# jankammeth/BA-path-planning

Hardware: AMD Instinct MI355X
Metric: SCP iterations/sec (N agents x K waypoints) (higher is better)
Workload: dtype f64

## Files before the change

ba-path-planning_amd/csrc/scp_common.h:

```cpp
#pragma once
#include <hip/hip_runtime.h>

#include <cstdarg>
#include <cstdint>
#include <cstdio>
#include <cstring>

#include "scp_hip.h"

struct scp_stats_mirror {
  scp_pair_stats stats;
  unsigned long long n_spec;
  double pts[6];
  double rel[64];
  volatile unsigned long long seq;
};

constexpr int SCP_SMALL_MAX_WG = 2048;

struct scp_ctx {
  int device;
  int n_cu;
  hipStream_t stream;
  char err[512];
// ... 35 lines not shown
    va_end(ap);
  }
  return code;
}

#define SCP_HIP_CHECK(ctx, call)                                                                     \
  do {                                                                                               \
    hipError_t e_ = (call);                                                                          \
    if (e_ != hipSuccess)                                                                            \
      return scp_fail((ctx), SCP_ERR_HIP, "%s failed: %s (%s:%d)", #call, hipGetErrorString(e_),    \
                      __FILE__, __LINE__);                                                           \
  } while (0)

#define SCP_REQUIRE(ctx, cond, ...)                                   \
  do {                                                                \
    if (!(cond)) return scp_fail((ctx), SCP_ERR_INVALID, __VA_ARGS__); \
  } while (0)

static inline int64_t scp_pairs(int N) { return (int64_t)N * (N - 1) / 2; }
static inline int scp_cdiv(int64_t a, int64_t b) { return (int)((a + b - 1) / b); }

hipError_t scp_raise_lds_limit(int device, const void* kernel, size_t bytes);

bool scp_wait_host_word(volatile unsigned long long* word, unsigned long long seq, int timeout_s);

int scp_ctx_wait_stats(scp_ctx* ctx, scp_pair_stats* out);

int scp_violations_from_solution(scp_ctx* ctx, int N, int K, int D, double R, double h, int64_t q_begin, int64_t q_end,
                                 const double* pos_prev, const double* x_tm, const double* p0, const double* v0, double* x_out,
                                 double* pos_out, double feas_tol, int64_t* new_rows, int64_t new_cap, uint32_t* sel_bitmap,
                                 scp_pair_stats* stats, const double* rel_prev ,
                                 int64_t* spec_rows , int64_t spec_cap,
                                 uint32_t* spec_bitmap, double spec_margin, bool* fused);
void scp_ctx_mirror_rel(scp_ctx* ctx, int64_t n, double* out);
int scp_select_from_solution(scp_ctx* ctx, int N, int K, int D, double R, double h, int64_t q_begin, int64_t q_end,
                             const double* x_tm, const double* p0, const double* v0, double* x_out, double* pos_out,
                             double margin, int64_t* sel_rows, int64_t sel_cap, uint32_t* sel_bitmap, scp_pair_stats* stats,
                             bool* fused);
int scp_launch_kinematics_copy(scp_ctx* ctx, int N, int K, int D, double h, const double* acc, const double* p0,
                               const double* v0, double* pos_out, double* vel_out, double* acc_copy);
const double* scp_qp_solution_tm(const scp_qp* qp);

int scp_qp_reset_add_rows_at(scp_qp* qp, const double* x0, int64_t n, const int64_t* rows, const double* pos_prev,
                             const double* p0, const double* v0, double R);
int scp_qp_add_rows_from_pass(scp_qp* qp, int64_t n, const int64_t* rows, const double* eta, const double* l_col,
                              int64_t q_begin, int64_t q_end);

int scp_launch_add_rows_at(scp_ctx* ctx, int N, int K, int D, int64_t base, int64_t n, const int64_t* rows,
                           const double* pos_prev, const double* p0, const double* v0, double R, double h, const double* Qx,
                           int64_t* w_row, int* wk, int* wi, int* wj, double* weta, double* wl, double* zc, double* yc);

int scp_launch_gemm(scp_ctx* ctx, int use_mfma, int R, int M, int C, double alpha, const double* A,
                    const double* X, double beta, double* Y);
int scp_launch_to_time_major(scp_ctx* ctx, int N, int K, int D, const double* src, double* dst);
int scp_launch_from_time_major(scp_ctx* ctx, int N, int K, int D, const double* src, double* dst);
int scp_launch_bounds_time_major(scp_ctx* ctx, int N, int K, int D, double h, const double* limits_host,
                                 const double* space_host, const double* p0, const double* v0,
                                 const double* pf, const double* vf, double* l_tm, double* u_tm,
                                 double* states_out );
```

ba-path-planning_amd/csrc/scp_kernels.hip:

```cpp
#include "scp_common.h"
#include "scp_pair_device.h"

#include <sys/prctl.h>
#include <time.h>

#include <atomic>
#include <chrono>
#include <cmath>
#include <cstdlib>
#include <map>
#include <mutex>
#include <type_traits>
#include <utility>

extern "C" int scp_abi_version(void) { return SCP_ABI_VERSION; }

extern "C" int scp_ctx_create(int device, void* hip_stream, scp_ctx** out) {
  if (!out) return SCP_ERR_INVALID;
  *out = nullptr;
  if (hipSetDevice(device) != hipSuccess) return SCP_ERR_HIP;
  scp_ctx* ctx = new scp_ctx();
  memset(ctx, 0, sizeof(*ctx));
  ctx->device = device;
  ctx->stream = (hipStream_t)hip_stream;
// ... 1280 lines not shown
#endif
}

static int ensure_tm(scp_ctx* ctx, size_t bytes) {
  if (ctx->tm_bytes >= bytes) return SCP_OK;
  if (ctx->tm_scratch) {
    SCP_HIP_CHECK(ctx, hipStreamSynchronize(ctx->stream));
    SCP_HIP_CHECK(ctx, hipFree(ctx->tm_scratch));
    ctx->tm_scratch = nullptr;
    ctx->tm_bytes = 0;
  }
  SCP_HIP_CHECK(ctx, hipMalloc(&ctx->tm_scratch, bytes));
  ctx->tm_bytes = bytes;
  return SCP_OK;
}

__global__ __launch_bounds__(256) void pair_prep_delta_kernel(int N, int K, int D, const double* __restrict__ pos_prev,
                                                               const double* __restrict__ pos_new,
                                                               double* __restrict__ P_tm, double* __restrict__ dP_tm,
                                                               scp_pair_stats* __restrict__ stats) {
  const int64_t t = (int64_t)blockIdx.x * 256 + threadIdx.x;
  const int64_t C = (int64_t)N * D;
  if (t == 0) pair_stats_init(stats);
  if (t >= C * K) return;
  const int k = (int)(t / C);
  const int c = (int)(t % C);
  const int i = c / D, d = c % D;
  const int64_t g = ((int64_t)i * K + k) * D + d;
  const double pp = pos_prev[g];
  P_tm[t] = pp;
  dP_tm[t] = pos_new[g] - pp;
}

struct PassTail {
  int64_t* rows;
  int64_t cap;
  uint32_t* merge_into;
  bool overwrite;
  int64_t words;
  bool done;
};

static bool small_pass_ok(const scp_ctx* ctx, int N, int K, int D, int64_t nq, int n_slices) {
  if (!ctx->small_pass || nq <= 0) return false;
  const int64_t words = (K * nq + 31) / 32;
  const int64_t n_wg = (int64_t)scp_cdiv(nq + 1, SMALL_ROWS) * K;
  return words <= CMP1_MAX_WORDS && (size_t)n_slices * N * D * sizeof(double) <= 32 * 1024 && n_wg <= SCP_SMALL_MAX_WG;
}

template <int MODE>
static int launch_pair_pass(scp_ctx* ctx, PairArgs& a, const double* pos_ref_layout, const double* p0,
                            const double* v0, uint32_t* clear_map = nullptr, int64_t clear_words = 0,
                            PassTail* tail = nullptr) {
  const int N = a.N, K = a.K, D = a.D;
  const int64_t nq = a.q_end - a.q_begin;
  if (tail) tail->done = false;
  if constexpr (MODE == MODE_SELECT || MODE == MODE_VIOL_RECOMPUTE || MODE == MODE_CHECK)
  if (tail) {
    const int n_slices = MODE == MODE_VIOL_RECOMPUTE ? (a.spec_rows ? 3 : 2) : 1;
    const size_t lds_small = (size_t)n_slices * N * D * sizeof(double);
    if (small_pass_ok(ctx, N, K, D, nq, n_slices)) {
      a.pos_a = pos_ref_layout;
      if (MODE == MODE_VIOL_RECOMPUTE && !a.x_tm) a.pos_b = p0;
      if (MODE != MODE_CHECK) {
        const size_t need = (size_t)(a.spec_rows ? 2 : 1) * scp_cdiv(nq + 1, SMALL_ROWS) * K * SMALL_ROWS * sizeof(uint32_t);
        if (ctx->wg_rows_bytes < need) {
          if (ctx->wg_rows) {
            SCP_HIP_CHECK(ctx, hipStreamSynchronize(ctx->stream));
            SCP_HIP_CHECK(ctx, hipFree(ctx->wg_rows));
            ctx->wg_rows = nullptr;
            ctx->wg_rows_bytes = 0;
          }
          SCP_HIP_CHECK(ctx, hipMalloc(&ctx->wg_rows, need));
          ctx->wg_rows_bytes = need;
        }
      }
      a.wg_rows = ctx->wg_rows;
      a.wg_part = ctx->wg_part;
      a.ticket = ctx->d_ticket;
      a.rows = tail->rows; a.cap = tail->cap; a.merge_into = tail->merge_into; a.overwrite = tail->overwrite ? 1 : 0;
      a.words = tail->words;
      a.mirror = ctx->d_mirror;
      a.seq = ++ctx->mirror_seq;
#ifdef SCP_PHASE_PROFILE
      a.ablate = getenv("SCP_PAIR_ABLATE") ? atoi(getenv("SCP_PAIR_ABLATE")) : 0;
#else
      a.ablate = 0;
#endif
      dim3 grid(scp_cdiv(nq + 1, SMALL_ROWS), K);
      if (ctx->timing) SCP_HIP_CHECK(ctx, hipEventRecord(ctx->pair_ev0, ctx->stream));
      if (D == 2) hipLaunchKernelGGL((pair_pass_kernel<2, MODE, true, true>), grid, dim3(PAIR_THREADS), lds_small, ctx->stream, a);
      else hipLaunchKernelGGL((pair_pass_kernel<3, MODE, true, true>), grid, dim3(PAIR_THREADS), lds_small, ctx->stream, a);
      SCP_HIP_CHECK(ctx, hipGetLastError());
      if (ctx->timing) SCP_HIP_CHECK(ctx, hipEventRecord(ctx->pair_ev1, ctx->stream));
      ctx->pair_timed = ctx->timing != 0;
      ctx->pair_ran = true;
      tail->done = true;
      ctx->last_pass_small = true;
      return SCP_OK;
    }
  }
  ctx->last_pass_small = false;
  const size_t slice = ((size_t)N * K * D + 1) & ~(size_t)1;
  int rc = ensure_tm(ctx, 2 * slice * sizeof(double));
  if (rc) return rc;
  double* P_tm = MODE != MODE_VIOLATIONS ? ctx->tm_scratch : nullptr;
  double* Q_tm = (MODE != MODE_CHECK && MODE != MODE_SELECT) ? ctx->tm_scratch + slice : nullptr;
  if (MODE == MODE_VIOL_RECOMPUTE)
    hipLaunchKernelGGL(pair_prep_delta_kernel, dim3(scp_cdiv((int64_t)N * K * D, 256)), dim3(256), 0, ctx->stream, N, K, D,
                       pos_ref_layout, p0, P_tm, Q_tm, a.stats);
  else
    hipLaunchKernelGGL(pair_prep_kernel, dim3(scp_cdiv((int64_t)N * K * D, 256)), dim3(256), 0, ctx->stream, N, K, D,
                       a.h, pos_ref_layout, p0, v0, P_tm, Q_tm, a.stats, clear_map, clear_words);
  a.P_tm = P_tm;
  a.Q_tm = Q_tm;
  if (nq <= 0) return SCP_OK;
  const size_t slice_bytes = (size_t)N * D * sizeof(double);
  const bool two_slices = MODE == MODE_LINEARIZE || MODE == MODE_VIOL_RECOMPUTE;
  const size_t lds_bytes = two_slices ? PAIR_LDS_SLICE_BYTES + slice_bytes : slice_bytes;
#ifdef SCP_PHASE_PROFILE
  const char* abl = getenv("SCP_PAIR_ABLATE");
  a.ablate = abl ? atoi(abl) : 0;
#else
  a.ablate = 0;
#endif
  const bool use_lds = slice_bytes <= (size_t)(two_slices ? 1 : 2) * PAIR_LDS_SLICE_BYTES && ((N * D) % 2 == 0) && !(a.ablate & 2);
  dim3 grid(scp_cdiv(nq + 1, PAIR_ROWS), K);
  dim3 block(PAIR_THREADS);
  if constexpr (MODE == MODE_LINEARIZE) {
    int per_cu = 0;
    const void* kern = D == 2 ? (use_lds ? (const void*)pair_pass_kernel<2, MODE_LINEARIZE, true> : (const void*)pair_pass_kernel<2, MODE_LINEARIZE, false>)
                              : (use_lds ? (const void*)pair_pass_kernel<3, MODE_LINEARIZE, true> : (const void*)pair_pass_kernel<3, MODE_LINEARIZE, false>);
    SCP_HIP_CHECK(ctx, hipOccupancyMaxActiveBlocksPerMultiprocessor(&per_cu, kern, PAIR_THREADS, use_lds ? lds_bytes : 0));
    const int64_t slots = (int64_t)std::max(per_cu, 1) * ctx->n_cu;
    PairItems& it = a.items;
    it = PairItems{};
    const int64_t big_per_k = scp_cdiv(nq + 1, PAIR_ROWS);
    int nk_quarter = 0, nk_half = 0;
    if (big_per_k * K > slots) {
      nk_quarter = (int)((slots * (PAIR_ROWS / 4) + nq / 2) / nq);
      nk_half = (int)((slots * (PAIR_ROWS / 2) + nq / 2) / nq);
// ... 486 lines not shown

int scp_violations_from_solution(scp_ctx* ctx, int N, int K, int D, double R, double h, int64_t q_begin, int64_t q_end,
                                 const double* pos_prev, const double* x_tm, const double* p0, const double* v0, double* x_out,
                                 double* pos_out, double feas_tol, int64_t* new_rows, int64_t new_cap, uint32_t* sel_bitmap,
                                 scp_pair_stats* stats, const double* rel_prev, int64_t* spec_rows, int64_t spec_cap,
                                 uint32_t* spec_bitmap, double spec_margin, bool* fused) {
  *fused = false;
  int rc = check_pair_range(ctx, N, K, D, q_begin, q_end);
  if (rc) return rc;
  const int64_t nq = q_end - q_begin;
  if (!small_pass_ok(ctx, N, K, D, nq, 2)) return SCP_OK;
  if (!spec_bitmap || !small_pass_ok(ctx, N, K, D, nq, 3)) spec_rows = nullptr;
  PairArgs a{};
  a.N = N; a.K = K; a.D = D; a.R = R; a.h = h;
  a.q_begin = q_begin; a.q_end = q_end; a.pairs = scp_pairs(N);
  a.margin = feas_tol;
  const int64_t words = (K * nq + 31) / 32;
  rc = ensure_cmp(ctx, words);
  if (rc) return rc;
  a.bitmap = sel_bitmap; a.mark = ctx->cmp_map; a.stats = stats;
  a.eta_stride = scp_eta_stride(K, nq);
  a.x_tm = x_tm; a.p0 = p0; a.v0 = v0; a.x_out = x_out; a.pos_out = pos_out;
  a.rel_prev = rel_prev;
  a.rel_blocks = rel_step_blocks((int64_t)N * K * D);
  a.spec_rows = spec_rows; a.spec_cap = spec_cap; a.spec_bitmap = spec_bitmap; a.spec_margin = spec_margin;
  PassTail tail{new_rows, new_cap, sel_bitmap, false, words, false};
  rc = launch_pair_pass<MODE_VIOL_RECOMPUTE>(ctx, a, pos_prev, nullptr, nullptr, nullptr, 0, &tail);
  if (rc) return rc;
  if (!tail.done) return scp_fail(ctx, SCP_ERR_STATE, "violations_from_solution: the small-problem pass did not run");
  *fused = true;
  return SCP_OK;
}

int scp_select_from_solution(scp_ctx* ctx, int N, int K, int D, double R, double h, int64_t q_begin, int64_t q_end,
                             const double* x_tm, const double* p0, const double* v0, double* x_out, double* pos_out,
                             double margin, int64_t* sel_rows, int64_t sel_cap, uint32_t* sel_bitmap, scp_pair_stats* stats,
                             bool* fused) {
  *fused = false;
  int rc = check_pair_range(ctx, N, K, D, q_begin, q_end);
  if (rc) return rc;
  const int64_t nq = q_end - q_begin;
  if (!small_pass_ok(ctx, N, K, D, nq, 1)) return SCP_OK;
  PairArgs a{};
  a.N = N; a.K = K; a.D = D; a.R = R; a.h = h;
  a.q_begin = q_begin; a.q_end = q_end; a.pairs = scp_pairs(N);
  a.margin = margin;
  a.bitmap = sel_bitmap; a.mark = sel_bitmap; a.stats = stats;
  a.eta_stride = scp_eta_stride(K, nq);
  a.x_tm = x_tm; a.p0 = p0; a.v0 = v0; a.x_out = x_out; a.pos_out = pos_out;
  PassTail tail{sel_rows, sel_cap, sel_bitmap, true, (K * nq + 31) / 32, false};
  rc = launch_pair_pass<MODE_SELECT>(ctx, a, nullptr, nullptr, nullptr, nullptr, 0, &tail);
  if (rc) return rc;
  if (!tail.done) return scp_fail(ctx, SCP_ERR_STATE, "select_from_solution: the small-problem pass did not run");
  *fused = true;
  return SCP_OK;
}

__global__ __launch_bounds__(256) void gather_rows_kernel(int64_t eta_stride, int D, int64_t pairs, int64_t q_begin, int64_t nq,
                                                           const double* __restrict__ eta,
                                                           const double* __restrict__ l,
                                                           const int64_t* __restrict__ rows, int64_t n,
                                                           double* __restrict__ w_eta, double* __restrict__ w_l) {
  const int64_t t = (int64_t)blockIdx.x * 256 + threadIdx.x;
  if (t >= n) return;
  const int64_t r = rows[t];
  const int64_t k = r / pairs, q = r % pairs;
// ... 80 lines not shown
```

ba-path-planning_amd/csrc/scp_qp.hip:

```cpp
#include "scp_qp_internal.h"
#include "scp_reset_device.h"

#include <chrono>
#include <cmath>
#include <vector>

__device__ inline double sum_partials(const double* part) {
  double s = 0.0;
  for (int b = 0; b < NPART; ++b) s += part[b];
  return s;
}

__global__ __launch_bounds__(256) void dot_partial_kernel(int64_t n, const double* __restrict__ a,
                                                           const double* __restrict__ b, double* __restrict__ part) {
  __shared__ double s[4];
  double acc = 0.0;
  for (int64_t t = (int64_t)blockIdx.x * 256 + threadIdx.x; t < n; t += (int64_t)NPART * 256) acc += a[t] * b[t];
#pragma unroll
  for (int o = 32; o > 0; o >>= 1) acc += __shfl_xor(acc, o);
  if ((threadIdx.x & 63) == 0) s[threadIdx.x >> 6] = acc;
  __syncthreads();
  if (threadIdx.x == 0) part[blockIdx.x] = (s[0] + s[1]) + (s[2] + s[3]);
}

// ... 308 lines not shown
  const int64_t r = rows[t];
  const int64_t k = r / pairs, q = r % pairs;
  const double b = 2.0 * N - 1.0;
  int64_t ii = (int64_t)((b - sqrt(b * b - 8.0 * (double)q)) * 0.5);
  if (ii < 0) ii = 0;
  if (ii > N - 2) ii = N - 2;
  while (ii * (2LL * N - ii - 1) / 2 > q) --ii;
  while (ii < N - 2 && (ii + 1) * (2LL * N - ii - 2) / 2 <= q) ++ii;
  const int64_t jj = q - ii * (2LL * N - ii - 1) / 2 + ii + 1;
  const int64_t o = base + t;
  w_row[o] = r;
  wk[o] = (int)k;
  wi[o] = (int)ii;
  wj[o] = (int)jj;
  const int64_t lr = k * nq + (q - q_begin);
  double ax = 0.0;
  for (int d = 0; d < D; ++d) {
    const double e = eta_stride ? eta_in[(int64_t)d * eta_stride + lr] : eta_in[t * D + d];
    weta[o * D + d] = e;
    ax += e * (Q[k * C + ii * D + d] - Q[k * C + jj * D + d]);
  }
  const double lo = eta_stride ? l_in[lr] : l_in[t];
  wl[o] = lo;
  zc[o] = fmax(ax, lo);
  yc[o] = 0.0;
}

__global__ __launch_bounds__(256) void qp_reset_kernel(int N, int K, int D, int Rf, const double* __restrict__ x0,
                                                        const double* __restrict__ F, const double* __restrict__ S0,
                                                        double* __restrict__ x, double* __restrict__ zf,
                                                        double* __restrict__ fx, double* __restrict__ Qx,
                                                        double* __restrict__ yf) {
  extern __shared__ double reset_xs[];
  qp_reset_body<false>(threadIdx.x, true, reset_xs, N, K, D, Rf, x0, F, S0, x, zf, fx, Qx, yf);
}

namespace {

inline size_t align_up(size_t v, size_t a = 256) { return (v + a - 1) / a * a; }

struct Carver {
  char* base;
  size_t off;
  template <typename T>
  T* take(size_t count) {
    T* p = base ? reinterpret_cast<T*>(base + off) : nullptr;
    off += align_up(count * sizeof(T));
    return p;
  }
};

size_t kkt_slot_doubles(int K) {
  auto al = [](size_t n) { return (n + 31) / 32 * 32; };
  return al((size_t)K * K) * 3 + al((size_t)2 * K * K) + 2 * al(scp_packed_count(K, K));
}

int kkt_slots(int K) {
  const size_t per = kkt_slot_doubles(K) * sizeof(double);
  const size_t fit = SCP_KKT_POOL_BYTES / per;
  return (int)std::min<size_t>(SCP_KKT_SLOTS_MAX, std::max<size_t>(SCP_KKT_SLOTS, fit));
}

size_t carve(QpDev& d, void* ws, int K, int64_t C, int64_t cap, int D) {
  const int Rf = 4 * K - 1;
  Carver c{static_cast<char*>(ws), 0};
  d.F = c.take<double>((size_t)Rf * K);
  d.Ft = c.take<double>((size_t)Rf * K);
// ... 412 lines not shown
  if (!qp) return SCP_ERR_INVALID;
  SCP_REQUIRE(qp->ctx, limits && space && p0 && v0 && pf && vf, "qp_set_problem: null pointer");
  QP_CHECK(scp_launch_bounds_time_major(qp->ctx, qp->N, qp->K, qp->D, qp->h, limits, space, p0, v0, pf, vf, qp->d.lf,
                                        qp->d.uf, qp->d.states));
  memcpy(qp->lim, limits, sizeof(qp->lim));
  for (int d = 0; d < 3; ++d) {
    qp->space[d] = d < qp->D ? space[d] : 0.0;
    qp->space[3 + d] = d < qp->D ? space[qp->D + d] : 0.0;
  }
  qp->problem_set = true;
  qp->reset_done = false;
  qp->persist_off = false;
  return SCP_OK;
}

struct RowsAt {
  const double *pos_prev, *p0, *v0;
  double R;
};

static int reset_impl(scp_qp* qp, const double* x0, int64_t n, const int64_t* rows, const RowsAt* at, bool* installed) {
  scp_ctx* ctx = qp->ctx;
  if (installed) *installed = false;
  if (!qp->problem_set) return scp_fail(ctx, SCP_ERR_STATE, "qp_reset: call scp_qp_set_problem first");
  const QpDev& d = qp->d;
  const int64_t nx = (int64_t)qp->K * qp->C, nf = (int64_t)qp->Rf * qp->C;
  const bool one_launch = qp->st.use_mfma == 1 && qp->K <= SCP_FUSED_MAX_K;
  qp->rho = qp->st.rho;
  bool with_rows = false;
  if (one_launch && at && ctx->small_pass && qp->st.cg_iters == 1 && n > 0 && n <= qp->row_cap)
    QP_CHECK(scp_qp_reset_install_small(qp, x0, n, rows, at->pos_prev, at->p0, at->v0, at->R, d.HQ + nx, &with_rows));
  if (with_rows) {
  } else if (one_launch) {
    hipLaunchKernelGGL(qp_reset_kernel, dim3(scp_cdiv(qp->C, RESET_COLS)), dim3(256),
                       (size_t)qp->K * RESET_COLS * sizeof(double), ctx->stream, qp->N, qp->K, qp->D, qp->Rf, x0, d.F, d.S0,
                       d.x, d.zf, d.fx, d.HQ + nx, d.yf);
    QP_LAUNCHED(qp);
  } else {
    if (x0) QP_CHECK(scp_launch_to_time_major(ctx, qp->N, qp->K, qp->D, x0, d.x));
    else SCP_HIP_CHECK(ctx, hipMemsetAsync(d.x, 0, nx * sizeof(double), ctx->stream));
    QP_CHECK(gemm(qp, qp->Rf, qp->K, 1.0, d.F, d.x, 0.0, d.zf));
    SCP_HIP_CHECK(ctx, hipMemsetAsync(d.yf, 0, nf * sizeof(double), ctx->stream));
  }
  qp->nW = with_rows ? n : 0;
  qp->persist_cap_nW = -1;
  qp->persist_off = false;
  qp->steps_since_reset = 0;
  qp_on_x_set(qp, one_launch);
  if (with_rows) qp_on_rows_added(qp, true);
  QP_CHECK(build_kkt(qp));
  qp->reset_done = true;
  if (installed) *installed = with_rows;
  return SCP_OK;
}

extern "C" int scp_qp_reset(scp_qp* qp, const double* x0) {
  if (!qp) return SCP_ERR_INVALID;
  return reset_impl(qp, x0, 0, nullptr, nullptr, nullptr);
}

extern "C" int scp_qp_set_rho(scp_qp* qp, double rho) {
  if (!qp) return SCP_ERR_INVALID;
  if (!qp->reset_done) return scp_fail(qp->ctx, SCP_ERR_STATE, "qp_set_rho: call scp_qp_reset first");
  SCP_REQUIRE(qp->ctx, rho >= 1e-6 && rho <= 1e6, "qp_set_rho: rho out of range");
  qp->rho = rho;
  qp_on_rho_changed(qp, false);
  return build_kkt(qp);
// ... 332 lines not shown
```

ba-path-planning_amd/csrc/scp_qp_fused.hip:

```cpp
#include "scp_qp_device.h"
#include "scp_pair_device.h"
#include "scp_reset_device.h"
#include <cstdlib>

namespace {

using namespace scpdev;
constexpr int FT = 1024;
constexpr int NWV = FT / 64;

#ifdef SCP_PHASE_PROFILE
__device__ unsigned long long scp_phase_clk[64];
#define PHASE_MARK(slot)                                                                      \
  do {                                                                                        \
    if (blockIdx.x == gridDim.x / 2 && threadIdx.x == 0) scp_phase_clk[slot] = wall_clock64(); \
  } while (0)
#else
#define PHASE_MARK(slot) ((void)0)
#endif

constexpr int SQ_BLOCKS = 128;
template <int E>
__global__ __launch_bounds__(FT) void cg1_col_kernel(int K, int Rf, int64_t C, double rho, double h,
                                                      const double* __restrict__ pMinv, const double* __restrict__ wrow,
// ... 646 lines not shown
constexpr int64_t CSR1_MAX_ROWS = 1 << 18;
struct CsrNewRows {
  int64_t n, base;
  const int64_t* rows;
  const double *pos_prev, *p0, *v0;
  double R, h;
  int N;
  int64_t* w_row;
  double* wl;
};
__global__ void csr_small_kernel(int64_t nW, int K, int ncell, int D, int64_t C, double rho, int* __restrict__ wk,
                                 int* __restrict__ wi, int* __restrict__ wj, double* __restrict__ weta,
                                 const double* __restrict__ Qx, double* __restrict__ zc, double* __restrict__ yc,
                                 int* __restrict__ ptr, int* __restrict__ ent, double* __restrict__ coef,
                                 int* __restrict__ pos_i, int* __restrict__ pos_j, double* __restrict__ gval, CsrNewRows nr);
}

int scp_qp_cg1_prepare(scp_qp* qp) {
  if (qp->dv.carried) return SCP_OK;
  const QpDev& d = qp->d;
  hipStream_t s = qp->ctx->stream;
  const int K = qp->K;
  const int64_t C = qp->C;
  const double rho_c = qp->rho * qp->st.rho_col_scale;
  QP_CHECK(scp_qp_exact_qx(qp, true));
  const double* Qx = scp_qp_qx(qp);
  if (qp->dv.vals_rho_c == rho_c) {
  } else if (!qp->dv.lists && qp->nW > 0 && qp->nW <= CSR1_MAX_ROWS && qp->N * K <= CSR1_MAX_CELLS) {
    const int ncell = qp->N * K;
    hipLaunchKernelGGL(csr_small_kernel, dim3(1), dim3(1024), (size_t)ncell * sizeof(int), s, qp->nW, K, ncell, qp->D, C, rho_c,
                       d.w_k, d.w_i, d.w_j, d.w_eta, Qx, d.zc, d.yc, d.cell_ptr, d.ent_code, d.coef, d.pos_i, d.pos_j, d.gval,
                       CsrNewRows{});
    FUSED_LAUNCHED(qp);
  } else {
    QP_CHECK(scp_qp_csr_ensure(qp));
    const dim3 rgrid((unsigned)((qp->nW + 255) / 256)), rblock(256);
    if (qp->D == 2)
      hipLaunchKernelGGL((rows_value_kernel<2, true>), rgrid, rblock, 0, s, qp->nW, C, rho_c, d.w_k, d.w_i, d.w_j, d.w_eta, Qx,
                         d.zc, d.yc, d.pos_i, d.pos_j, d.gval);
    else
      hipLaunchKernelGGL((rows_value_kernel<3, true>), rgrid, rblock, 0, s, qp->nW, C, rho_c, d.w_k, d.w_i, d.w_j, d.w_eta, Qx,
                         d.zc, d.yc, d.pos_i, d.pos_j, d.gval);
    FUSED_LAUNCHED(qp);
  }
  qp_on_cg1_prepared(qp);
  return SCP_OK;
}

int scp_qp_install_rows_small(scp_qp* qp, int64_t n, const int64_t* rows, const double* pos_prev, const double* p0,
                              const double* v0, double R, const double* Qx, bool* done) {
  *done = false;
  const QpDev& d = qp->d;
  const int K = qp->K;
  const int64_t nW = qp->nW + n;
  if (!qp->dv.qx || n <= 0 || nW > CSR1_MAX_ROWS || qp->N * K > CSR1_MAX_CELLS) return SCP_OK;
  const int ncell = qp->N * K;
  const double rho_c = qp->rho * qp->st.rho_col_scale;
  CsrNewRows nr{n, qp->nW, rows, pos_prev, p0, v0, R, qp->h, qp->N, d.w_row, d.w_l};
  hipLaunchKernelGGL(csr_small_kernel, dim3(1), dim3(1024), (size_t)ncell * sizeof(int), qp->ctx->stream, nW, K, ncell, qp->D,
                     qp->C, rho_c, d.w_k, d.w_i, d.w_j, d.w_eta, Qx, d.zc, d.yc, d.cell_ptr, d.ent_code, d.coef, d.pos_i,
                     d.pos_j, d.gval, nr);
  FUSED_LAUNCHED(qp);
  *done = true;
  return SCP_OK;
}

// ... 101 lines not shown
#pragma unroll
  for (int e = 0; e < SCAN_SC; ++e) {
    if (c + e < ncell) ptr[c + e] = run;
    run += v[e];
  }
  if (threadIdx.x == 255) blk_tot[blockIdx.x] = run;
}

__global__ __launch_bounds__(256) void csr_scan_add_kernel(int ncell, int nblk, int* __restrict__ ptr, int* __restrict__ cur,
                                                            const int* __restrict__ blk_tot) {
  int off = 0;
  for (int b = 0; b < (int)blockIdx.x; ++b) off += blk_tot[b];
  const int c = blockIdx.x * SCAN_CELLS + SCAN_SC * (int)threadIdx.x;
#pragma unroll
  for (int e = 0; e < SCAN_SC; ++e) {
    if (c + e < ncell) {
      const int v = ptr[c + e] + off;
      ptr[c + e] = v;
      cur[c + e] = v;
    }
  }
  if (blockIdx.x == nblk - 1 && threadIdx.x == 0) ptr[ncell] = off + blk_tot[nblk - 1];
}

__global__ __launch_bounds__(256) void csr_fill_kernel(int64_t nW, int K, const int* __restrict__ wk,
                                                        const int* __restrict__ wi, const int* __restrict__ wj,
                                                        int* __restrict__ cur, int* __restrict__ ent) {
  const int64_t n = (int64_t)blockIdx.x * 256 + threadIdx.x;
  if (n >= nW) return;
  ent[atomicAdd(cur + cell_of(wk[n], wi[n], K), 1)] = (int)(2 * n);
  ent[atomicAdd(cur + cell_of(wk[n], wj[n], K), 1)] = (int)(2 * n + 1);
}

__global__ __launch_bounds__(256) void csr_sort_kernel(int ncell, const int* __restrict__ ptr, int* __restrict__ ent) {
  const int c = blockIdx.x * 256 + threadIdx.x;
  if (c >= ncell) return;
  const int b = ptr[c], e = ptr[c + 1];
  for (int i = b + 1; i < e; ++i) {
    const int v = ent[i];
    int j = i - 1;
    while (j >= b && ent[j] > v) {
      ent[j + 1] = ent[j];
      --j;
    }
    ent[j + 1] = v;
  }
}

__global__ __launch_bounds__(256) void csr_finish_kernel(int64_t nent, int D, const int* __restrict__ ent,
                                                          const double* __restrict__ weta, double* __restrict__ coef,
                                                          int* __restrict__ pos_i, int* __restrict__ pos_j) {
  const int64_t t = (int64_t)blockIdx.x * 256 + threadIdx.x;
  if (t >= nent) return;
  const int code = ent[t];
  const int n = code >> 1, side = code & 1;
  for (int d = 0; d < D; ++d) coef[t * D + d] = side ? -weta[(int64_t)n * D + d] : weta[(int64_t)n * D + d];
  if (side) pos_j[n] = (int)t;
  else pos_i[n] = (int)t;
}

template <bool COH>
__device__ inline void csr_small_body(int* csr_cnt, int64_t nW, int K, int ncell, int D, int64_t C, double rho,
                                                          int* __restrict__ wk, int* __restrict__ wi,
                                                          int* __restrict__ wj, double* __restrict__ weta,
                                                          const double* __restrict__ Qx, double* __restrict__ zc,
                                                          double* __restrict__ yc, int* __restrict__ ptr,
                                                          int* __restrict__ ent, double* __restrict__ coef,
                                                          int* __restrict__ pos_i, int* __restrict__ pos_j,
                                                          double* __restrict__ gval, CsrNewRows nr) {
  __shared__ int wsum[16];
  constexpr int SC = CSR1_MAX_CELLS / 1024;
  const int tid = threadIdx.x, lane = tid & 63, wave = tid >> 6;
  if (nr.n > 0) {
    const int64_t pairs = (int64_t)nr.N * (nr.N - 1) / 2;
    for (int64_t t = tid; t < nr.n; t += 1024) {
      if (D == 2)
        add_row_at<2, COH>(t, nr.N, K, C, pairs, nr.base, nr.rows, nr.pos_prev, nr.p0, nr.v0, nr.R, nr.h, Qx, nr.w_row, wk, wi, wj,
                      weta, nr.wl, zc, yc);
      else
        add_row_at<3, COH>(t, nr.N, K, C, pairs, nr.base, nr.rows, nr.pos_prev, nr.p0, nr.v0, nr.R, nr.h, Qx, nr.w_row, wk, wi, wj,
                      weta, nr.wl, zc, yc);
    }
    __threadfence_block();
    __syncthreads();
  }
  for (int c = tid; c < ncell; c += 1024) csr_cnt[c] = 0;
  __syncthreads();
  for (int64_t n = tid; n < nW; n += 1024) {
    atomicAdd(&csr_cnt[cell_of(wk[n], wi[n], K)], 1);
    atomicAdd(&csr_cnt[cell_of(wk[n], wj[n], K)], 1);
  }
// ... 130 lines not shown
                                                          const double* __restrict__ yc, const double* __restrict__ vec,
                                                          const int* __restrict__ pos_i, const int* __restrict__ pos_j,
                                                          double* __restrict__ gval, const double* __restrict__ vec2,
                                                          double* __restrict__ gval2) {
  const int64_t n = (int64_t)blockIdx.x * 256 + threadIdx.x;
  if (n >= nW) return;
  if (gval2) {
    const double g2 = vec2[n];
    gval2[pos_i[n]] = g2;
    gval2[pos_j[n]] = g2;
  }
  const double g = mode == 0 ? rho * zc[n] - yc[n] : (mode == 1 ? yc[n] : vec[n]);
  gval[pos_i[n]] = g;
  gval[pos_j[n]] = g;
}

__global__ __launch_bounds__(256) void csr_gather_kernel(int K, int N, int D, const int* __restrict__ ptr,
                                                          const double* __restrict__ coef,
                                                          const double* __restrict__ gval, double* __restrict__ G) {
  const int64_t t = (int64_t)blockIdx.x * 256 + threadIdx.x;
  const int64_t C = (int64_t)N * D;
  if (t >= C * K) return;
  const int k = (int)(t / C), col = (int)(t % C);
  const int agent = col / D, d = col - agent * D;
  const int cell = cell_of(k, agent, K);
  double acc = 0.0;
  const int t1 = ptr[cell + 1];
  for (int e = ptr[cell]; e < t1; ++e) acc += coef[(size_t)e * D + d] * gval[e];
  G[t] = acc;
}

}

int scp_qp_csr_ensure(scp_qp* qp) {
  if (qp->dv.lists) return SCP_OK;
  const QpDev& d = qp->d;
  hipStream_t s = qp->ctx->stream;
  const int ncell = qp->N * qp->K;
  SCP_REQUIRE(qp->ctx, 2 * qp->nW < 0x3FFFFFFF, "csr_build: too many working rows for 32-bit entry codes");
  SCP_HIP_CHECK(qp->ctx, hipMemsetAsync(d.cell_ptr, 0, (size_t)(ncell + 1) * sizeof(int), s));
  if (qp->nW > 0) {
    const dim3 rgrid((unsigned)((qp->nW + 255) / 256));
    hipLaunchKernelGGL(csr_count_kernel, rgrid, dim3(256), 0, s, qp->nW, qp->K, d.w_k, d.w_i, d.w_j, d.cell_ptr);
    const int sblk = (ncell + SCAN_CELLS - 1) / SCAN_CELLS;
    hipLaunchKernelGGL(csr_scan_local_kernel, dim3(sblk), dim3(256), 0, s, ncell, d.cell_ptr, d.scan_tot);
    hipLaunchKernelGGL(csr_scan_add_kernel, dim3(sblk), dim3(256), 0, s, ncell, sblk, d.cell_ptr, d.cell_cur, d.scan_tot);
    hipLaunchKernelGGL(csr_fill_kernel, rgrid, dim3(256), 0, s, qp->nW, qp->K, d.w_k, d.w_i, d.w_j, d.cell_cur, d.ent_code);
    hipLaunchKernelGGL(csr_sort_kernel, dim3((ncell + 255) / 256), dim3(256), 0, s, ncell, d.cell_ptr, d.ent_code);
    hipLaunchKernelGGL(csr_finish_kernel, dim3((unsigned)((2 * qp->nW + 255) / 256)), dim3(256), 0, s, 2 * qp->nW, qp->D,
                       d.ent_code, d.w_eta, d.coef, d.pos_i, d.pos_j);
    FUSED_LAUNCHED(qp);
  }
  qp_on_lists_built(qp);
  return SCP_OK;
}

int scp_qp_csr_scatter(scp_qp* qp, int mode, const double* vec) {
  QP_CHECK(scp_qp_csr_ensure(qp));
  const QpDev& d = qp->d;
  hipStream_t s = qp->ctx->stream;
  const int64_t nx = (int64_t)qp->K * qp->C;
  hipLaunchKernelGGL(csr_rowval_kernel, dim3((unsigned)((qp->nW + 255) / 256)), dim3(256), 0, s, qp->nW, mode,
                     qp->rho * qp->st.rho_col_scale, d.zc, d.yc, vec, d.pos_i, d.pos_j, d.gval, (const double*)nullptr, (double*)nullptr);
  hipLaunchKernelGGL(csr_gather_kernel, dim3((unsigned)((nx + 255) / 256)), dim3(256), 0, s, qp->K, qp->N, qp->D,
                     d.cell_ptr, d.coef, d.gval, d.G);
  FUSED_LAUNCHED(qp);
  return SCP_OK;
}

int scp_qp_rows_gather(scp_qp* qp, const double* Q) {
  const QpDev& d = qp->d;
  hipStream_t s = qp->ctx->stream;
  QP_CHECK(scp_qp_csr_ensure(qp));
  const int64_t C = qp->C, nx = (int64_t)qp->K * C;
  const double rho_c = qp->rho * qp->st.rho_col_scale;
  const dim3 rgrid((unsigned)((qp->nW + 255) / 256)), rblock(256);
  if (qp->D == 2)
    hipLaunchKernelGGL((rows_value_kernel<2, false>), rgrid, rblock, 0, s, qp->nW, C, rho_c, d.w_k, d.w_i, d.w_j, d.w_eta, Q,
                       d.zc, d.yc, d.pos_i, d.pos_j, d.gval);
  else
    hipLaunchKernelGGL((rows_value_kernel<3, false>), rgrid, rblock, 0, s, qp->nW, C, rho_c, d.w_k, d.w_i, d.w_j, d.w_eta, Q,
                       d.zc, d.yc, d.pos_i, d.pos_j, d.gval);
  hipLaunchKernelGGL(csr_gather_kernel, dim3((unsigned)((nx + 255) / 256)), dim3(256), 0, s, qp->K, qp->N, qp->D,
// ... 345 lines not shown
```

ba-path-planning_amd/csrc/scp_qp_internal.h:

```cpp
#pragma once
#include "scp_common.h"

constexpr int SCP_KKT_SLOTS = 6;
constexpr int SCP_KKT_SLOTS_MAX = 32;
constexpr size_t SCP_KKT_POOL_BYTES = (size_t)48 << 20;
constexpr int NPART = 128;

#define QP_CHECK(call)            \
  do {                            \
    int rc_ = (call);             \
    if (rc_ != SCP_OK) return rc_; \
  } while (0)

enum Slot {
  SL_RZ0 = 0, SL_RZ1 = 1,
  SL_RP = 8, SL_NAX = 9, SL_NZ = 10, SL_RD = 11, SL_NPX = 12, SL_NATY = 13,
  SL_NDY = 14, SL_SUPP = 15, SL_NATDY = 16,
  SL_COUNT = 32
};

struct QpDev {
  double *F, *Ft, *S0, *S0t, *HS, *Hf, *Minv, *aug, *wrow;
  double* gj_tmp;
  double* G0;
// ... 61 lines not shown
  double lim[6];
  int64_t steps_since_reset;
  int persist_variant;
  int persist_fault;
  bool persist_off;
  bool persist_skip_solve;
  int persist_gave_up_total;
  int64_t persist_cap_nW;
  int persist_cap;
  unsigned long long persist_epoch;
  unsigned* h_persist;
  int persist_rho_switches;
  double persist_rho;
  unsigned* h_persist_dev;
};

constexpr int64_t SCP_FINE_MAX_COLUMNS = 4096;
inline int scp_qp_fine_cadence(const scp_qp* qp) {
  const scp_qp_settings& st = qp->st;
  const bool fine = st.check_fine > 0 && st.check_fine < st.check_termination && st.check_termination % st.check_fine == 0 &&
                    qp->nW > 0 && qp->C <= SCP_FINE_MAX_COLUMNS;
  return fine ? st.check_fine : 0;
}

constexpr int SCP_RESID_STRIDE = 12;
constexpr int SCP_RESID_CAP = (4096 / 2 + 128) * SCP_RESID_STRIDE;
constexpr int SCP_INV_LDS_MAX_K = 96;
constexpr int SCP_BIGK_MAX_K = 1024;
constexpr int SCP_FUSED_MAX_K = 120;
constexpr int SCP_PART_CAP = 4096;
int scp_qp_cg1_iteration(scp_qp* qp, int* cg_count, bool emit_dy);
int scp_qp_qp0_iterations(scp_qp* qp, int nit, double* dy_out);
int scp_qp_csr_scatter(scp_qp* qp, int mode, const double* vec);
int scp_qp_csr_ensure(scp_qp* qp);
int scp_qp_rows_gather(scp_qp* qp, const double* Q);
int scp_qp_cg1_prepare(scp_qp* qp);
int scp_qp_exact_qx(scp_qp* qp, bool with_fx);
inline double* scp_qp_qx(const scp_qp* qp, bool other = false) {
  return (qp->dv.qx_half != 0) != other ? qp->d.HQ : qp->d.HQ + (int64_t)qp->K * qp->C;
}
int scp_qp_install_rows_small(scp_qp* qp, int64_t n, const int64_t* rows, const double* pos_prev, const double* p0,
                              const double* v0, double R, const double* Qx, bool* done);
int scp_qp_reset_install_small(scp_qp* qp, const double* x0, int64_t n, const int64_t* rows, const double* pos_prev,
                               const double* p0, const double* v0, double R, double* Qx, bool* done);
constexpr int SCP_SYNC_WORDS = 16;
constexpr int SCP_PERSIST_MAX_WG = 256;
constexpr int SCP_GPART_WORDS = 2 * (SCP_PERSIST_MAX_WG + 1) * 4;
constexpr int SCP_GCHECK_WORDS = (SCP_PERSIST_MAX_WG + 1) * 9 * 2;
bool scp_qp_persist_eligible(const scp_qp* qp);
bool scp_persist_claim(int device, int n_cu_total, int n_wg, int wait_ms);
void scp_persist_release(int device, int n_wg);
constexpr int SCP_PERSIST_GAVE_UP = 2;
int scp_qp_cg1_persist(scp_qp* qp, int it0, int cad0, int* ran, int* code, int* it_done);
int scp_qp_pack_operands(scp_qp* qp);
static inline size_t scp_packed_count(int R, int M) { return (size_t)((R + 15) / 16) * ((M + 3) / 4) * 64; }
int scp_qp_fused_residuals(scp_qp* qp, bool with_dy);

inline void qp_on_x_set(scp_qp* qp, bool qx) {
  QpDerived& v = qp->dv;
  v.lists = v.carried = false; v.vals_rho_c = 0.0; v.qx = qx;
  if (qx) v.qx_half = 0;
}
inline void qp_on_rows_added(scp_qp* qp, bool small_install) {
  qp->dv.lists = small_install; qp->dv.vals_rho_c = small_install ? qp->rho * qp->st.rho_col_scale : 0.0;
  qp->dv.carried = false;
}
inline void qp_on_rho_changed(scp_qp* qp, bool in_kernel) { qp->dv.vals_rho_c = 0.0; qp->dv.carried &= in_kernel; }
// ... 12 lines not shown
```

ba-path-planning_amd/csrc/scp_reset_device.h:

```cpp
#pragma once
#include <hip/hip_runtime.h>

#include <cstdint>

#include "scp_pair_device.h"

constexpr int RESET_COLS = 16;
template <bool COH>
__device__ inline void qp_reset_body(int tid, bool active, double* reset_xs, int N, int K, int D, int Rf,
                                     const double* __restrict__ x0, const double* __restrict__ F,
                                     const double* __restrict__ S0, double* __restrict__ x, double* __restrict__ zf,
                                     double* __restrict__ fx, double* __restrict__ Qx, double* __restrict__ yf) {
  constexpr int RG = 256 / RESET_COLS;
  const int64_t C = (int64_t)N * D;
  const int lc = tid & (RESET_COLS - 1), rg = tid / RESET_COLS;
  const int64_t c = (int64_t)blockIdx.x * RESET_COLS + lc;
  const bool live = active && c < C;
  const int64_t agent = live ? c / D : 0;
  const int dim = live ? (int)(c - agent * D) : 0;
  if (active) {
    for (int k = rg; k < K; k += RG) {
      const double v = (live && x0) ? x0[(agent * K + k) * D + dim] : 0.0;
      reset_xs[k * RESET_COLS + lc] = v;
      if (live) x[(int64_t)k * C + c] = v;
    }
  }
  __syncthreads();
  if (!active) return;
  constexpr int RB = 4;
  for (int r0 = rg * RB; r0 < Rf + K; r0 += RG * RB) {
    const double* __restrict__ row[RB];
    double acc[RB];
#pragma unroll
    for (int j = 0; j < RB; ++j) {
      const int r = min(r0 + j, Rf + K - 1);
      row[j] = r < Rf ? F + (size_t)r * K : S0 + (size_t)(r - Rf) * K;
      acc[j] = 0.0;
    }
#pragma unroll 2
    for (int k = 0; k < K; ++k) {
      const double xv = reset_xs[k * RESET_COLS + lc];
#pragma unroll
      for (int j = 0; j < RB; ++j) acc[j] += row[j][k] * xv;
    }
    if (!live) continue;
#pragma unroll
    for (int j = 0; j < RB; ++j) {
      const int r = r0 + j;
      if (r >= Rf + K) break;
      if (r < Rf) {
        zf[(int64_t)r * C + c] = acc[j];
        fx[(int64_t)r * C + c] = acc[j];
        yf[(int64_t)r * C + c] = 0.0;
      } else if (COH) {
        store_coherent(Qx + (int64_t)(r - Rf) * C + c, acc[j]);
      } else {
        Qx[(int64_t)(r - Rf) * C + c] = acc[j];
      }
    }
  }
}
```

ba-path-planning_amd/csrc/scp_solver.hip:

```cpp
#include "scp_common.h"

#include <chrono>
#include <cmath>
#include <cstdlib>
#include <vector>

struct StepState {
  const double *limits, *space, *p0, *v0, *pf, *vf;
  const double* acc_in;
  scp_solve_options o;
  double eps;
  int64_t q_begin, q_end;
  bool row_free;
  int max_iter, used, rounds;
  int64_t nW, last_added;
  double max_v;
  float lin_ms, viol_ms;
  scp_qp_info info;
  scp_qp_settings saved;
  bool active;
  bool fuse_ok;
  bool solution_pending;
  bool rel_ready;
  bool spec_ok;
// ... 222 lines not shown
  SV_CHECK(scp_qp_get_solution(s->qp, s->x));
  return scp_kinematics(s->ctx, s->N, s->K, s->D, s->h, s->x, t.p0, t.v0, s->pos_b, nullptr);
}

int step_violations(scp_solver* s, StepState& t, int64_t* n_new) {
  scp_ctx* ctx = s->ctx;
  *n_new = 0;
  if (t.q_end <= t.q_begin) {
    if (t.solution_pending) SV_CHECK(materialise_solution(s, t));
    t.max_v = -INFINITY;
    return SCP_OK;
  }
  for (;;) {
    if (t.solution_pending) {
      bool fused = false;
      const bool spec = s->want_spec && t.row_free && t.q_begin == 0 && t.q_end == s->pairs;
      if (spec && !s->sel2) {
        const size_t words = (size_t)std::max<int64_t>((s->rows + 31) / 32, 1);
        SV_HIP(hipMalloc(&s->sel2, (size_t)s->sel_cap * sizeof(int64_t)));
        s->sel2_cap = s->sel_cap;
        SV_HIP(hipMalloc(&s->bitmap2, words * sizeof(uint32_t)));
      }
      SV_CHECK(scp_violations_from_solution(ctx, s->N, s->K, s->D, s->R, s->h, t.q_begin, t.q_end, s->pos_a,
                                            scp_qp_solution_tm(s->qp), t.p0, t.v0, s->x, s->pos_b, t.o.feasibility_tol,
                                            s->sel, s->sel_cap, s->bitmap, s->stats, t.acc_in, spec ? s->sel2 : nullptr,
                                            s->sel2_cap, s->bitmap2, t.o.working_set_margin, &fused));
      t.solution_pending = false;
      if (fused) {
        SV_CHECK(read_stats(s, true));
        scp_ctx_mirror_rel(ctx, (int64_t)s->N * s->K * s->D, t.rel);
        t.rel_ready = true;
        t.spec_n = (int64_t)ctx->h_mirror->n_spec;
        t.spec_ok = spec && t.spec_n > 0 && t.spec_n <= s->sel2_cap;
        if ((int64_t)s->h_stats->n_selected <= s->sel_cap) break;
        SV_CHECK(grow_sel(s, (int64_t)s->h_stats->n_selected));
        continue;
      }
      SV_CHECK(scp_qp_get_solution(s->qp, s->x));
      SV_CHECK(scp_kinematics(ctx, s->N, s->K, s->D, s->h, s->x, t.p0, t.v0, s->pos_b, nullptr));
    }
    SV_CHECK(scp_collision_violations_at(ctx, s->N, s->K, s->D, s->R, t.q_begin, t.q_end, s->pos_a, s->pos_b,
                                         t.o.feasibility_tol, s->sel, s->sel_cap, s->bitmap, s->stats));
    SV_CHECK(read_stats(s, true));
    if ((int64_t)s->h_stats->n_selected <= s->sel_cap) break;
    SV_CHECK(grow_sel(s, (int64_t)s->h_stats->n_selected));
  }
  SV_CHECK(scp_ctx_last_pair_ms(ctx, &t.viol_ms));
  *n_new = (int64_t)s->h_stats->n_selected;
  t.max_v = s->h_stats->max_violation;
  return SCP_OK;
}

bool step_round_done(StepState& t, int64_t n_all, scp_qp_record* rec) {
  if (t.rounds < SCP_MAX_ROUNDS_RECORDED) rec->added[t.rounds] = n_all;
  ++t.rounds;
  t.last_added = n_all;
  return !(n_all == 0 || t.used >= t.max_iter || t.rounds >= t.o.max_rounds);
}

void step_finish(scp_solver* s, StepState& t, scp_qp_record* rec) {
  rec->status_val = t.info.status_val;
  rec->working_rows = t.info.working_rows;
  rec->r_prim = t.info.r_prim;
  rec->r_dual = t.info.r_dual;
  rec->rho = t.info.rho;
  rec->rounds = t.rounds;
// ... 373 lines not shown
```

Measured before the change: 416.0.

## Fuse solution kinematics into violation pass, merge CSR finish, split reset rows

Adds a pair-prep kernel that computes kinematics from the time-major QP solution and writes x, positions and the delta arrays in one launch. The violation check can then skip the separate get_solution and kinematics launches when the small-pass path is enabled. The CSR sort and finish kernels are merged into one, which can also precompute gval from Qx. The QP reset kernel's row loop is split across a 2D grid for more parallelism, which makes each block redundantly load the x0 tile into LDS.

```diff
diff --git a/ba-path-planning_amd/csrc/scp_common.h b/ba-path-planning_amd/csrc/scp_common.h
--- a/ba-path-planning_amd/csrc/scp_common.h
+++ b/ba-path-planning_amd/csrc/scp_common.h
@@ -91,6 +91,10 @@
                                  scp_pair_stats* stats, const double* rel_prev ,
                                  int64_t* spec_rows , int64_t spec_cap,
                                  uint32_t* spec_bitmap, double spec_margin, bool* fused);
+int scp_violations_at_solution(scp_ctx* ctx, int N, int K, int D, double R, double h, int64_t q_begin, int64_t q_end,
+                               const double* pos_prev, const double* x_tm, const double* p0, const double* v0, double* x_out,
+                               double* pos_out, double feas_tol, int64_t* new_rows, int64_t new_cap, uint32_t* sel_bitmap,
+                               scp_pair_stats* stats, bool* done);
 void scp_ctx_mirror_rel(scp_ctx* ctx, int64_t n, double* out);
 int scp_select_from_solution(scp_ctx* ctx, int N, int K, int D, double R, double h, int64_t q_begin, int64_t q_end,
                              const double* x_tm, const double* p0, const double* v0, double* x_out, double* pos_out,
diff --git a/ba-path-planning_amd/csrc/scp_kernels.hip b/ba-path-planning_amd/csrc/scp_kernels.hip
--- a/ba-path-planning_amd/csrc/scp_kernels.hip
+++ b/ba-path-planning_amd/csrc/scp_kernels.hip
@@ -1336,6 +1336,35 @@
   dP_tm[t] = pos_new[g] - pp;
 }
 
+__global__ __launch_bounds__(256) void pair_prep_solution_kernel(int N, int K, int D, double h, const double* __restrict__ x_tm,
+                                                                  const double* __restrict__ p0, const double* __restrict__ v0,
+                                                                  const double* __restrict__ pos_prev,
+                                                                  double* __restrict__ x_out, double* __restrict__ pos_out,
+                                                                  double* __restrict__ P_tm, double* __restrict__ dP_tm,
+                                                                  scp_pair_stats* __restrict__ stats) {
+  const int64_t t = (int64_t)blockIdx.x * 256 + threadIdx.x;
+  const int64_t C = (int64_t)N * D;
+  if (t == 0) pair_stats_init(stats);
+  if (t >= C * K) return;
+  const int k = (int)(t / C);
+  const int c = (int)(t % C);
+  const int i = c / D, d = c % D;
+  const int64_t g = ((int64_t)i * K + k) * D + d;
+  double pn, vn;
+  kin_point(x_tm + c, C, k, h, p0[c], v0[c], pn, vn);
+  x_out[g] = x_tm[t];
+  pos_out[g] = pn;
+  const double pp = pos_prev[g];
+  P_tm[t] = pp;
+  dP_tm[t] = pn - pp;
+}
+
+struct PassSolution {
+  const double *x_tm, *p0, *v0;
+  double h;
+  double *x_out, *pos_out;
+};
+
 struct PassTail {
   int64_t* rows;
   int64_t cap;
@@ -1355,7 +1384,7 @@
 template <int MODE>
 static int launch_pair_pass(scp_ctx* ctx, PairArgs& a, const double* pos_ref_layout, const double* p0,
                             const double* v0, uint32_t* clear_map = nullptr, int64_t clear_words = 0,
-                            PassTail* tail = nullptr) {
+                            PassTail* tail = nullptr, const PassSolution* sol = nullptr) {
   const int N = a.N, K = a.K, D = a.D;
   const int64_t nq = a.q_end - a.q_begin;
   if (tail) tail->done = false;
@@ -1410,7 +1439,10 @@
   if (rc) return rc;
   double* P_tm = MODE != MODE_VIOLATIONS ? ctx->tm_scratch : nullptr;
   double* Q_tm = (MODE != MODE_CHECK && MODE != MODE_SELECT) ? ctx->tm_scratch + slice : nullptr;
-  if (MODE == MODE_VIOL_RECOMPUTE)
+  if (MODE == MODE_VIOL_RECOMPUTE && sol)
+    hipLaunchKernelGGL(pair_prep_solution_kernel, dim3(scp_cdiv((int64_t)N * K * D, 256)), dim3(256), 0, ctx->stream, N, K, D,
+                       sol->h, sol->x_tm, sol->p0, sol->v0, pos_ref_layout, sol->x_out, sol->pos_out, P_tm, Q_tm, a.stats);
+  else if (MODE == MODE_VIOL_RECOMPUTE)
     hipLaunchKernelGGL(pair_prep_delta_kernel, dim3(scp_cdiv((int64_t)N * K * D, 256)), dim3(256), 0, ctx->stream, N, K, D,
                        pos_ref_layout, p0, P_tm, Q_tm, a.stats);
   else
@@ -1963,6 +1995,32 @@
   return SCP_OK;
 }
 
+int scp_violations_at_solution(scp_ctx* ctx, int N, int K, int D, double R, double h, int64_t q_begin, int64_t q_end,
+                               const double* pos_prev, const double* x_tm, const double* p0, const double* v0, double* x_out,
+                               double* pos_out, double feas_tol, int64_t* new_rows, int64_t new_cap, uint32_t* sel_bitmap,
+                               scp_pair_stats* stats, bool* done) {
+  *done = false;
+  if (!ctx->small_pass) return SCP_OK;
+  int rc = check_pair_range(ctx, N, K, D, q_begin, q_end);
+  if (rc) return rc;
+  PairArgs a{};
+  a.N = N; a.K = K; a.D = D; a.R = R; a.h = 0.0;
+  a.q_begin = q_begin; a.q_end = q_end; a.pairs = scp_pairs(N);
+  a.margin = feas_tol;
+  const int64_t nq = q_end - q_begin;
+  const int64_t words = (K * nq + 31) / 32;
+  rc = ensure_cmp(ctx, words);
+  if (rc) return rc;
+  a.bitmap = sel_bitmap; a.mark = ctx->cmp_map; a.stats = stats;
+  a.eta_stride = scp_eta_stride(K, nq);
+  const PassSolution sol{x_tm, p0, v0, h, x_out, pos_out};
+  rc = launch_pair_pass<MODE_VIOL_RECOMPUTE>(ctx, a, pos_prev, nullptr, nullptr, nullptr, 0, nullptr, &sol);
+  if (rc) return rc;
+  *done = true;
+  if (nq <= 0) return SCP_OK;
+  return launch_compaction(ctx, ctx->cmp_map, words, nq, q_begin, a.pairs, new_rows, new_cap, sel_bitmap, stats);
+}
+
 int scp_select_from_solution(scp_ctx* ctx, int N, int K, int D, double R, double h, int64_t q_begin, int64_t q_end,
                              const double* x_tm, const double* p0, const double* v0, double* x_out, double* pos_out,
                              double margin, int64_t* sel_rows, int64_t sel_cap, uint32_t* sel_bitmap, scp_pair_stats* stats,
diff --git a/ba-path-planning_amd/csrc/scp_qp.hip b/ba-path-planning_amd/csrc/scp_qp.hip
--- a/ba-path-planning_amd/csrc/scp_qp.hip
+++ b/ba-path-planning_amd/csrc/scp_qp.hip
@@ -364,7 +364,7 @@
                                                         double* __restrict__ fx, double* __restrict__ Qx,
                                                         double* __restrict__ yf) {
   extern __shared__ double reset_xs[];
-  qp_reset_body<false>(threadIdx.x, true, reset_xs, N, K, D, Rf, x0, F, S0, x, zf, fx, Qx, yf);
+  qp_reset_body<false>(threadIdx.x, true, reset_xs, N, K, D, Rf, x0, F, S0, x, zf, fx, Qx, yf, blockIdx.y, gridDim.y);
 }
 
 namespace {
@@ -843,7 +843,7 @@
     QP_CHECK(scp_qp_reset_install_small(qp, x0, n, rows, at->pos_prev, at->p0, at->v0, at->R, d.HQ + nx, &with_rows));
   if (with_rows) {
   } else if (one_launch) {
-    hipLaunchKernelGGL(qp_reset_kernel, dim3(scp_cdiv(qp->C, RESET_COLS)), dim3(256),
+    hipLaunchKernelGGL(qp_reset_kernel, dim3(scp_cdiv(qp->C, RESET_COLS), scp_cdiv(qp->Rf + qp->K, RESET_PASS_ROWS)), dim3(256),
                        (size_t)qp->K * RESET_COLS * sizeof(double), ctx->stream, qp->N, qp->K, qp->D, qp->Rf, x0, d.F, d.S0,
                        d.x, d.zf, d.fx, d.HQ + nx, d.yf);
     QP_LAUNCHED(qp);
diff --git a/ba-path-planning_amd/csrc/scp_qp_fused.hip b/ba-path-planning_amd/csrc/scp_qp_fused.hip
--- a/ba-path-planning_amd/csrc/scp_qp_fused.hip
+++ b/ba-path-planning_amd/csrc/scp_qp_fused.hip
@@ -702,6 +702,8 @@
                        d.w_k, d.w_i, d.w_j, d.w_eta, Qx, d.zc, d.yc, d.cell_ptr, d.ent_code, d.coef, d.pos_i, d.pos_j, d.gval,
                        CsrNewRows{});
     FUSED_LAUNCHED(qp);
+  } else if (!qp->dv.lists && qp->nW > 0) {
+    QP_CHECK(scp_qp_csr_ensure(qp, Qx));
   } else {
     QP_CHECK(scp_qp_csr_ensure(qp));
     const dim3 rgrid((unsigned)((qp->nW + 255) / 256)), rblock(256);
@@ -869,7 +871,14 @@
   ent[atomicAdd(cur + cell_of(wk[n], wj[n], K), 1)] = (int)(2 * n + 1);
 }
 
-__global__ __launch_bounds__(256) void csr_sort_kernel(int ncell, const int* __restrict__ ptr, int* __restrict__ ent) {
+template <int D>
+__global__ __launch_bounds__(256) void csr_sort_finish_kernel(int ncell, int64_t C, double rho, const int* __restrict__ ptr,
+                                                               int* __restrict__ ent, const int* __restrict__ wk,
+                                                               const int* __restrict__ wi, const int* __restrict__ wj,
+                                                               const double* __restrict__ weta, double* __restrict__ coef,
+                                                               int* __restrict__ pos_i, int* __restrict__ pos_j,
+                                                               const double* __restrict__ Q, const double* __restrict__ zc,
+                                                               const double* __restrict__ yc, double* __restrict__ gval) {
   const int c = blockIdx.x * 256 + threadIdx.x;
   if (c >= ncell) return;
   const int b = ptr[c], e = ptr[c + 1];
@@ -882,18 +891,23 @@
     }
     ent[j + 1] = v;
   }
-}
-
-__global__ __launch_bounds__(256) void csr_finish_kernel(int64_t nent, int D, const int* __restrict__ ent,
-                                                          const double* __restrict__ weta, double* __restrict__ coef,
-                                                          int* __restrict__ pos_i, int* __restrict__ pos_j) {
-  const int64_t t = (int64_t)blockIdx.x * 256 + threadIdx.x;
-  if (t >= nent) return;
-  const int code = ent[t];
-  const int n = code >> 1, side = code & 1;
-  for (int d = 0; d < D; ++d) coef[t * D + d] = side ? -weta[(int64_t)n * D + d] : weta[(int64_t)n * D + d];
-  if (side) pos_j[n] = (int)t;
-  else pos_i[n] = (int)t;
+  for (int t = b; t < e; ++t) {
+    const int code = ent[t];
+    const int64_t n = code >> 1;
+    const int side = code & 1;
+#pragma unroll
+    for (int d = 0; d < D; ++d) coef[(int64_t)t * D + d] = side ? -weta[n * D + d] : weta[n * D + d];
+    if (side) pos_j[n] = t;
+    else pos_i[n] = t;
+    if (Q) {
+      const int64_t bi = (int64_t)wk[n] * C + (int64_t)wi[n] * D;
+      const int64_t bj = (int64_t)wk[n] * C + (int64_t)wj[n] * D;
+      double ax = 0.0;
+#pragma unroll
+      for (int d = 0; d < D; ++d) ax += weta[n * D + d] * (Q[bi + d] - Q[bj + d]);
+      gval[t] = (rho * zc[n] - yc[n]) - rho * ax;
+    }
+  }
 }
 
 template <bool COH>
@@ -1090,7 +1104,7 @@
 
 }
 
-int scp_qp_csr_ensure(scp_qp* qp) {
+int scp_qp_csr_ensure(scp_qp* qp, const double* Qx_vals) {
   if (qp->dv.lists) return SCP_OK;
   const QpDev& d = qp->d;
   hipStream_t s = qp->ctx->stream;
@@ -1104,9 +1118,13 @@
     hipLaunchKernelGGL(csr_scan_local_kernel, dim3(sblk), dim3(256), 0, s, ncell, d.cell_ptr, d.scan_tot);
     hipLaunchKernelGGL(csr_scan_add_kernel, dim3(sblk), dim3(256), 0, s, ncell, sblk, d.cell_ptr, d.cell_cur, d.scan_tot);
     hipLaunchKernelGGL(csr_fill_kernel, rgrid, dim3(256), 0, s, qp->nW, qp->K, d.w_k, d.w_i, d.w_j, d.cell_cur, d.ent_code);
-    hipLaunchKernelGGL(csr_sort_kernel, dim3((ncell + 255) / 256), dim3(256), 0, s, ncell, d.cell_ptr, d.ent_code);
-    hipLaunchKernelGGL(csr_finish_kernel, dim3((unsigned)((2 * qp->nW + 255) / 256)), dim3(256), 0, s, 2 * qp->nW, qp->D,
-                       d.ent_code, d.w_eta, d.coef, d.pos_i, d.pos_j);
+    const double rho_c = qp->rho * qp->st.rho_col_scale;
+    if (qp->D == 2)
+      hipLaunchKernelGGL(csr_sort_finish_kernel<2>, dim3((ncell + 255) / 256), dim3(256), 0, s, ncell, qp->C, rho_c, d.cell_ptr,
+                         d.ent_code, d.w_k, d.w_i, d.w_j, d.w_eta, d.coef, d.pos_i, d.pos_j, Qx_vals, d.zc, d.yc, d.gval);
+    else
+      hipLaunchKernelGGL(csr_sort_finish_kernel<3>, dim3((ncell + 255) / 256), dim3(256), 0, s, ncell, qp->C, rho_c, d.cell_ptr,
+                         d.ent_code, d.w_k, d.w_i, d.w_j, d.w_eta, d.coef, d.pos_i, d.pos_j, Qx_vals, d.zc, d.yc, d.gval);
     FUSED_LAUNCHED(qp);
   }
   qp_on_lists_built(qp);
diff --git a/ba-path-planning_amd/csrc/scp_qp_internal.h b/ba-path-planning_amd/csrc/scp_qp_internal.h
--- a/ba-path-planning_amd/csrc/scp_qp_internal.h
+++ b/ba-path-planning_amd/csrc/scp_qp_internal.h
@@ -117,7 +117,7 @@
 int scp_qp_cg1_iteration(scp_qp* qp, int* cg_count, bool emit_dy);
 int scp_qp_qp0_iterations(scp_qp* qp, int nit, double* dy_out);
 int scp_qp_csr_scatter(scp_qp* qp, int mode, const double* vec);
-int scp_qp_csr_ensure(scp_qp* qp);
+int scp_qp_csr_ensure(scp_qp* qp, const double* Qx_vals = nullptr);
 int scp_qp_rows_gather(scp_qp* qp, const double* Q);
 int scp_qp_cg1_prepare(scp_qp* qp);
 int scp_qp_exact_qx(scp_qp* qp, bool with_fx);
diff --git a/ba-path-planning_amd/csrc/scp_reset_device.h b/ba-path-planning_amd/csrc/scp_reset_device.h
--- a/ba-path-planning_amd/csrc/scp_reset_device.h
+++ b/ba-path-planning_amd/csrc/scp_reset_device.h
@@ -6,11 +6,13 @@
 #include "scp_pair_device.h"
 
 constexpr int RESET_COLS = 16;
+constexpr int RESET_PASS_ROWS = 256 / RESET_COLS * 4;
 template <bool COH>
 __device__ inline void qp_reset_body(int tid, bool active, double* reset_xs, int N, int K, int D, int Rf,
                                      const double* __restrict__ x0, const double* __restrict__ F,
                                      const double* __restrict__ S0, double* __restrict__ x, double* __restrict__ zf,
-                                     double* __restrict__ fx, double* __restrict__ Qx, double* __restrict__ yf) {
+                                     double* __restrict__ fx, double* __restrict__ Qx, double* __restrict__ yf,
+                                     int part = 0, int n_parts = 1) {
   constexpr int RG = 256 / RESET_COLS;
   const int64_t C = (int64_t)N * D;
   const int lc = tid & (RESET_COLS - 1), rg = tid / RESET_COLS;
@@ -22,13 +24,14 @@
     for (int k = rg; k < K; k += RG) {
       const double v = (live && x0) ? x0[(agent * K + k) * D + dim] : 0.0;
       reset_xs[k * RESET_COLS + lc] = v;
-      if (live) x[(int64_t)k * C + c] = v;
+      if (live && part == 0) x[(int64_t)k * C + c] = v;
     }
   }
   __syncthreads();
   if (!active) return;
   constexpr int RB = 4;
-  for (int r0 = rg * RB; r0 < Rf + K; r0 += RG * RB) {
+  static_assert(RG * RB == RESET_PASS_ROWS, "qp_reset_kernel's grid assumes this pass height");
+  for (int r0 = (part * RG + rg) * RB; r0 < Rf + K; r0 += n_parts * RG * RB) {
     const double* __restrict__ row[RB];
     double acc[RB];
 #pragma unroll
diff --git a/ba-path-planning_amd/csrc/scp_solver.hip b/ba-path-planning_amd/csrc/scp_solver.hip
--- a/ba-path-planning_amd/csrc/scp_solver.hip
+++ b/ba-path-planning_amd/csrc/scp_solver.hip
@@ -278,6 +278,16 @@
         t.rel_ready = true;
         t.spec_n = (int64_t)ctx->h_mirror->n_spec;
         t.spec_ok = spec && t.spec_n > 0 && t.spec_n <= s->sel2_cap;
+        if ((int64_t)s->h_stats->n_selected <= s->sel_cap) break;
+        SV_CHECK(grow_sel(s, (int64_t)s->h_stats->n_selected));
+        continue;
+      }
+      bool done = false;
+      SV_CHECK(scp_violations_at_solution(ctx, s->N, s->K, s->D, s->R, s->h, t.q_begin, t.q_end, s->pos_a,
+                                          scp_qp_solution_tm(s->qp), t.p0, t.v0, s->x, s->pos_b, t.o.feasibility_tol, s->sel,
+                                          s->sel_cap, s->bitmap, s->stats, &done));
+      if (done) {
+        SV_CHECK(read_stats(s, true));
         if ((int64_t)s->h_stats->n_selected <= s->sel_cap) break;
         SV_CHECK(grow_sel(s, (int64_t)s->h_stats->n_selected));
         continue;
```

Result: faster. 423.1 (median of 6 runs) (+1.7%).
